# ShioMisaka/fce-yolo

Hardware: AMD Instinct MI355X
Metric: images/sec/GPU @ 640x640 bs=32, yolo11n-fce; fraction of fp16 MFMA roofline (higher is better)
Workload: dtype fp16; 1 GPU; yolo11n-fce detection inference (forward + decode + NMS) @ 640x640, 32 images/GPU; model=yolo11n-fce, global_batch=32, imgsz=640, parallelism=dp1, batches_in_flight=4, distinct_inputs=5, hw_queues=8, forward_launch=hipgraph

## Files before the change

### fce-yolo_amd/csrc/detect_cls.hip

```cpp
#include <algorithm>

#include "mfma_stage.h"

namespace fce {

static __device__ __attribute__((aligned(16))) _Float16 g_dc_zero[8];

constexpr int dc_max(int a, int b) { return a > b ? a : b; }

template <int C0, int C3, int NCLS, int TH, int TW, int NW>
struct DcG {
  static constexpr int NT = NW * 64;
  static constexpr int K0 = C0 / 8, K3 = C3 / 8;
  static constexpr int XW = TW + 4, XR = (TH + 4) * XW;
  static constexpr int RW = TW + 2, R1 = (TH + 2) * RW;
  static constexpr int NC = TH * TW;
  static constexpr int sX = K0, s1 = K0 | 1, s3 = K3 | 1;
  static constexpr int NF1 = (R1 + 15) / 16, NF2 = (NC + 15) / 16;
  static constexpr int MF1 = (NF1 + NW - 1) / NW, MF2 = (NF2 + NW - 1) / NW;
  static constexpr int CT3 = (C3 + 15) / 16, CTN = (NCLS + 15) / 16;
  static constexpr int NS1 = (K0 + 3) / 4, NS2 = (K3 + 3) / 4;
  static constexpr int W1 = CT3 * NS1 * 64, W2 = CT3 * NS2 * 64, W3 = CTN * NS2 * 64;
  static constexpr int OW2 = W1, OW3 = W1 + W2, OD = W1 + W2 + W3;
  static constexpr int ND = 9 * (C0 + C3);
  static constexpr int BD1 = 0, BP1 = C0, BD2 = BP1 + CT3 * 16, BP2 = BD2 + C3, BC = BP2 + CT3 * 16, NB = BC + CTN * 16;
  static constexpr int OB = OD + ND / 4;
  static constexpr int OP = OB + (NB + 3) / 4;
  static constexpr int PSZ = dc_max(R1 * s1, NC * s3);
  static constexpr int OQ = OP + PSZ;
  static constexpr int QX = XR * K0, QT = R1 * K3;
  static constexpr int QSZ = dc_max(dc_max(2 * QX, 2 * QT), NC * s3);
  static constexpr int TOTAL = OQ + QSZ;
  static constexpr size_t LDS = size_t(TOTAL) * 16;
  static constexpr int NXE = (XR * K0 + NT - 1) / NT;
  static constexpr int NPG3 = NT / K3;
  static constexpr int MINB = (LDS <= 80 * 1024 && NW == 4) ? 2 : 1;
  static_assert(C0 % 8 == 0 && C3 % 8 == 0 && NT % K0 == 0 && NPG3 > 0, "detect cls fused: channel alignment");
};

struct DclsArgs {
  const _Float16* x;
  int xcs;
  int H, W, tiles_x, tiles_y, ntiles;
  const float* dw[2];
  const h8* pw[3];
  int nalloc[3];
  const float* b[5];
  float* pred;
  unsigned long long* best;
  int A, a0;
  int diag;
};

__device__ __forceinline__ void dc_tile(const DclsArgs& a, int TH, int TW, int t, int& n, int& y0, int& x0) {
  const int tx = t % a.tiles_x;
  t /= a.tiles_x;
  const int ty = t % a.tiles_y;
  n = t / a.tiles_y;
  y0 = ty * TH;
  x0 = tx * TW;
}

typedef float f2 __attribute__((ext_vector_type(2)));
__device__ __forceinline__ h8 dc_dw(const f4* img, int plane, int p00, int rw, int k, int ch, int iy, int H,
                                    const float (&wk)[9][8], const float (&bz)[8]) {
  f2 acc[4];
#pragma unroll
  for (int j = 0; j < 4; ++j) acc[j] = f2{bz[2 * j], bz[2 * j + 1]};
#pragma unroll
  for (int ky = 0; ky < 3; ++ky) {
    const int yy = iy - 1 + ky;
    if (yy < 0 || yy >= H) continue;
#pragma unroll
    for (int kx = 0; kx < 3; ++kx) {
      const int u = (p00 + ky * rw + kx) * k + ch;
      const f4 lo = img[u], hi = img[plane + u];
      const float* w = wk[ky * 3 + kx];
      acc[0] = __builtin_elementwise_fma(f2{lo[0], lo[1]}, f2{w[0], w[1]}, acc[0]);
      acc[1] = __builtin_elementwise_fma(f2{lo[2], lo[3]}, f2{w[2], w[3]}, acc[1]);
      acc[2] = __builtin_elementwise_fma(f2{hi[0], hi[1]}, f2{w[4], w[5]}, acc[2]);
      acc[3] = __builtin_elementwise_fma(f2{hi[2], hi[3]}, f2{w[6], w[7]}, acc[3]);
    }
  }
  h8 o;
#pragma unroll
  for (int j = 0; j < 8; ++j) o[j] = (_Float16)fpin(silu(acc[j >> 1][j & 1]));
  return o;
}

__device__ __forceinline__ void dc_weights(const float* tab, int c, int ch, const float* bias, float (&wk)[9][8],
                                           float (&bz)[8]) {
#pragma unroll
  for (int t = 0; t < 9; ++t) {
    const f4 w0 = *reinterpret_cast<const f4*>(tab + t * c + ch * 8);
    const f4 w1 = *reinterpret_cast<const f4*>(tab + t * c + ch * 8 + 4);
#pragma unroll
    for (int j = 0; j < 4; ++j) {
      wk[t][j] = w0[j];
      wk[t][j + 4] = w1[j];
    }
  }
  const f4 b0 = *reinterpret_cast<const f4*>(bias + ch * 8);
  const f4 b1 = *reinterpret_cast<const f4*>(bias + ch * 8 + 4);
#pragma unroll
  for (int j = 0; j < 4; ++j) {
    bz[j] = b0[j];
    bz[j + 4] = b1[j];
  }
}

template <int C0, int C3, int NCLS, int TH, int TW, int NW>
__global__ __launch_bounds__(NW * 64, (DcG<C0, C3, NCLS, TH, TW, NW>::MINB)) void detect_cls_fused_kernel(DclsArgs a) {
  using G = DcG<C0, C3, NCLS, TH, TW, NW>;
  extern __shared__ __attribute__((aligned(16))) h8 sm[];
  const int tid = threadIdx.x, lane = tid & 63, wave = tid >> 6, col = lane & 15, grp = lane >> 4;
  const int NG = gridDim.x, bi = blockIdx.x;
  const int t_begin = int(int64_t(bi) * a.ntiles / NG), t_end = int(int64_t(bi + 1) * a.ntiles / NG);
  if (t_begin >= t_end) return;

  h8 xr[G::NXE];
  auto load_x = [&](int t) {
    int n, y0, x0;
    dc_tile(a, TH, TW, t, n, y0, x0);
#pragma unroll
    for (int k = 0; k < G::NXE; ++k) {
      const int e = tid + k * G::NT, pos = e / G::K0, ch = e - pos * G::K0;
      const int r = pos / G::XW, c = pos - r * G::XW;
      const int iy = y0 - 2 + r, ix = x0 - 2 + c;
      const bool in = pos < G::XR && iy >= 0 && iy < a.H && ix >= 0 && ix < a.W;
      const _Float16* src = in ? a.x + nhwc_off(n, iy, ix, a.H, a.W, a.xcs) + ch * 8 : g_dc_zero;
      xr[k] = *reinterpret_cast<const h8*>(src);
    }
  };
  load_x(t_begin);
  {
    stage_copy_frags(sm, a.pw[0], G::CT3, G::NS1, a.nalloc[0], G::NT);
    stage_copy_frags(sm + G::OW2, a.pw[1], G::CT3, G::NS2, a.nalloc[1], G::NT);
    stage_copy_frags(sm + G::OW3, a.pw[2], G::CTN, G::NS2, a.nalloc[2], G::NT);
    float* d = reinterpret_cast<float*>(sm + G::OD);
    for (int e = tid; e < 9 * C0; e += G::NT) d[e] = a.dw[0][e];
    for (int e = tid; e < 9 * C3; e += G::NT) d[9 * C0 + e] = a.dw[1][e];
    float* bs = reinterpret_cast<float*>(sm + G::OB);
    for (int e = tid; e < G::NB; e += G::NT) {
      float v;
      if (e < G::BP1) v = a.b[0][e];
      else if (e < G::BD2) v = e - G::BP1 < C3 ? a.b[1][e - G::BP1] : 0.f;
      else if (e < G::BP2) v = a.b[2][e - G::BD2];
      else if (e < G::BC) v = e - G::BP2 < C3 ? a.b[3][e - G::BP2] : 0.f;
      else v = e - G::BC < NCLS ? a.b[4][e - G::BC] : 0.f;
      bs[e] = v;
    }
  }
  __syncthreads();

  const float* dwt = reinterpret_cast<const float*>(sm + G::OD);
  const float* bias = reinterpret_cast<const float*>(sm + G::OB);
  h8* P = sm + G::OP;
  h8* Q = sm + G::OQ;
  _Float16* Qh = reinterpret_cast<_Float16*>(Q);
  f4* Qf = reinterpret_cast<f4*>(Q);
  const h8 zero8 = {0, 0, 0, 0, 0, 0, 0, 0};
  uint64_t clk[7] = {0, 0, 0, 0, 0, 0, 0}, tprev = a.diag ? __builtin_amdgcn_s_memtime() : 0;
  auto tick = [&](int k) {
    if (a.diag) {
      const uint64_t tn = __builtin_amdgcn_s_memtime();
      clk[k] += tn - tprev;
      tprev = tn;
    }
  };

  for (int t = t_begin; t < t_end; ++t) {
    int n, y0, x0;
    dc_tile(a, TH, TW, t, n, y0, x0);
#pragma unroll
    for (int k = 0; k < G::NXE; ++k) {
      const int e = tid + k * G::NT, pos = e / G::K0;
      if (pos < G::XR) {
        const h8 v = xr[k];
        Qf[e] = f4{(float)v[0], (float)v[1], (float)v[2], (float)v[3]};
        Qf[G::QX + e] = f4{(float)v[4], (float)v[5], (float)v[6], (float)v[7]};
      }
    }
    tick(0);
    if (t + 1 < t_end) load_x(t + 1);
    stage_barrier();
    tick(1);
    {
      const int ch = tid % G::K0;
      float wk[9][8], bz[8];
      dc_weights(dwt, C0, ch, bias + G::BD1, wk, bz);
      for (int pos = tid / G::K0; pos < G::R1; pos += G::NT / G::K0) {
        const int r = pos / G::RW, c = pos - r * G::RW;
        const int iy = y0 - 1 + r, ix = x0 - 1 + c;
        h8 o = zero8;
        if (iy >= 0 && iy < a.H && ix >= 0 && ix < a.W) o = dc_dw(Qf, G::QX, r * G::XW + c, G::XW, G::K0, ch, iy, a.H, wk, bz);
        P[pos * G::s1 + ch] = o;
      }
    }
    stage_barrier();
    tick(2);
    {
      int pq[G::MF1];
#pragma unroll
      for (int i = 0; i < G::MF1; ++i) pq[i] = min((wave + NW * i) * 16 + col, G::R1 - 1) * G::s1;
      auto bl = [&](int i, int st) -> h8 {
        const int cc = st * 4 + grp;
        return cc < G::K0 ? P[pq[i] + cc] : zero8;
      };
      auto epi = [&](int i, int ct, const f4& acc) {
        const int q = (wave + NW * i) * 16 + col, co0 = ct * 16 + grp * 4;
        if (q >= G::R1 || co0 >= C3) return;
        const int r = q / G::RW, c = q - r * G::RW;
        const int iy = y0 - 1 + r, ix = x0 - 1 + c;
        float v[4];
#pragma unroll
        for (int j = 0; j < 4; ++j) v[j] = silu(acc[j] + bias[G::BP1 + co0 + j]);
        const h4 o = h4_of(v);
        const bool in = iy >= 0 && iy < a.H && ix >= 0 && ix < a.W;
        Qf[(co0 & 4 ? G::QT : 0) + q * G::K3 + (co0 >> 3)] =
            in ? f4{(float)o[0], (float)o[1], (float)o[2], (float)o[3]} : f4{0.f, 0.f, 0.f, 0.f};
      };
      mfma_stage<G::MF1, G::CT3, G::NS1>(sm + lane, bl, epi);
    }
    stage_barrier();
    tick(3);
    if (tid < G::NPG3 * G::K3) {
      const int ch = tid % G::K3;
      float wk[9][8], bz[8];
      dc_weights(dwt + 9 * C0, C3, ch, bias + G::BD2, wk, bz);
      for (int pos = tid / G::K3; pos < G::NC; pos += G::NPG3) {
        const int r = pos / TW, c = pos - r * TW;
        const int iy = y0 + r, ix = x0 + c;
        h8 o = zero8;
        if (iy < a.H && ix < a.W) o = dc_dw(Qf, G::QT, r * G::RW + c, G::RW, G::K3, ch, iy, a.H, wk, bz);
        P[pos * G::s3 + ch] = o;
      }
    }
    stage_barrier();
    tick(4);
    {
      int pq[G::MF2];
#pragma unroll
      for (int i = 0; i < G::MF2; ++i) pq[i] = min((wave + NW * i) * 16 + col, G::NC - 1) * G::s3;
      auto bl = [&](int i, int st) -> h8 {
        const int cc = st * 4 + grp;
        return cc < G::K3 ? P[pq[i] + cc] : zero8;
      };
      auto epi = [&](int i, int ct, const f4& acc) {
        const int q = (wave + NW * i) * 16 + col, co0 = ct * 16 + grp * 4;
        if (q >= G::NC || co0 >= C3) return;
        float v[4];
#pragma unroll
        for (int j = 0; j < 4; ++j) v[j] = silu(acc[j] + bias[G::BP2 + co0 + j]);
        *reinterpret_cast<h4*>(Qh + (q * G::s3) * 8 + co0) = h4_of(v);
      };
      mfma_stage<G::MF2, G::CT3, G::NS2>(sm + G::OW2 + lane, bl, epi);
    }
    stage_barrier();
    tick(5);
    {
      int pq[G::MF2];
#pragma unroll
      for (int i = 0; i < G::MF2; ++i) pq[i] = min((wave + NW * i) * 16 + col, G::NC - 1) * G::s3;
      unsigned long long bk[G::MF2];
#pragma unroll
      for (int i = 0; i < G::MF2; ++i) bk[i] = 0ull;
      auto bl = [&](int i, int st) -> h8 {
        const int cc = st * 4 + grp;
        return cc < G::K3 ? Q[pq[i] + cc] : zero8;
      };
      auto epi = [&](int i, int ct, const f4& acc) {
        const int q = (wave + NW * i) * 16 + col, co0 = ct * 16 + grp * 4;
        if (q >= G::NC) return;
        const int r = q / TW, c = q - r * TW;
        const int iy = y0 + r, ix = x0 + c;
        if (iy >= a.H || ix >= a.W) return;
        float* o = a.pred + (int64_t(n) * (4 + NCLS) + 4 + co0) * a.A + a.a0 + iy * a.W + ix;
        const int nv = min(4, NCLS - co0);
#pragma unroll
        for (int j = 0; j < 4; ++j)
          if (j < nv) {
            const float sc = sigmoidf_(acc[j] + bias[G::BC + co0 + j]);
            o[int64_t(j) * a.A] = sc;
            const unsigned long long key =
                (uint64_t(__float_as_uint(sc)) << 32) | uint64_t(0xFFFFFFFFu - uint32_t(co0 + j));
            bk[i] = key > bk[i] ? key : bk[i];
          }
      };
      mfma_stage<G::MF2, G::CTN, G::NS2>(sm + G::OW3 + lane, bl, epi);
      if (a.best) {
#pragma unroll
        for (int i = 0; i < G::MF2; ++i) {
          unsigned long long k = bk[i];
          const unsigned long long k16 = __shfl_xor(k, 16);
          k = k16 > k ? k16 : k;
          const unsigned long long k32 = __shfl_xor(k, 32);
          k = k32 > k ? k32 : k;
          const int q = (wave + NW * i) * 16 + col;
          const int r = q / TW, c = q - r * TW;
          if (grp == 0 && q < G::NC && y0 + r < a.H && x0 + c < a.W && k)
            atomicMax(a.best + int64_t(n) * a.A + a.a0 + (y0 + r) * a.W + x0 + c, k);
        }
      }
    }
    stage_barrier();
    tick(6);
  }
  if (a.diag && blockIdx.x == 0 && threadIdx.x == 0) {
    const unsigned long long nt = (unsigned long long)(t_end - t_begin);
    printf("detect cls fused diag: %llu tiles, clocks per tile: x->lds %llu, x-issue+barrier %llu, dw1 %llu, pw1 %llu, "
           "dw2 %llu, pw2 %llu, cls %llu\n", nt, (unsigned long long)clk[0] / nt, (unsigned long long)clk[1] / nt,
           (unsigned long long)clk[2] / nt, (unsigned long long)clk[3] / nt, (unsigned long long)clk[4] / nt,
           (unsigned long long)clk[5] / nt, (unsigned long long)clk[6] / nt);
  }
}

struct DcInst {
  int c0, c3, nc;
};
static constexpr DcInst kDcInsts[] = {{64, 80, 80}, {128, 80, 80}};

template <int C0, int C3, int NCLS, int TH, int TW, int NW>
static int dc_launch(const DclsArgs& a0, int N, hipStream_t s) {
  using G = DcG<C0, C3, NCLS, TH, TW, NW>;
  static_assert(G::LDS <= 160 * 1024, "detect cls fused: LDS over 160 KiB");
  auto k = detect_cls_fused_kernel<C0, C3, NCLS, TH, TW, NW>;
  static const bool big = hipFuncSetAttribute(reinterpret_cast<const void*>(k),
                                              hipFuncAttributeMaxDynamicSharedMemorySize, 160 * 1024) == hipSuccess;
  if (!big && G::LDS > 64 * 1024) return fail(FCE_ERR_HIP, "detect cls fused: cannot opt in to >64 KiB LDS");
  DclsArgs a = a0;
  a.tiles_x = (a.W + TW - 1) / TW;
  a.tiles_y = (a.H + TH - 1) / TH;
  const int64_t tiles = int64_t(a.tiles_x) * a.tiles_y * N;
  if (tiles == 0) return FCE_OK;
  FCE_CHECK(tiles < (int64_t(1) << 30), "detect cls fused: grid too large");
  a.ntiles = int(tiles);
  static int cus = 0;
  if (!cus) {
    int dev = 0;
    if (hipGetDevice(&dev) != hipSuccess || hipDeviceGetAttribute(&cus, hipDeviceAttributeMultiprocessorCount, dev) != hipSuccess)
      cus = 256;
  }
  int occ = 0;
  if (hipOccupancyMaxActiveBlocksPerMultiprocessor(&occ, k, G::NT, G::LDS) != hipSuccess || occ < 1) occ = 1;
  const int grid = int(std::min<int64_t>(a.ntiles, int64_t(cus) * occ));
  FCE_LAUNCH(k, dim3(unsigned(grid)), dim3(G::NT), G::LDS, s, a);
  return launch_status("detect_cls_fused_kernel");
}

static bool dc_tile_env(const char* name, const char* v) {
  const char* e = getenv(name);
  return e && strcmp(e, v) == 0;
}

static int dc_dispatch(int inst, const DclsArgs& a, int N, hipStream_t s) {
  const char* name = inst == 0 ? "FCE_DCLS_TILE_64" : "FCE_DCLS_TILE_128";
  const char* env = getenv(name);
  const bool set = env && *env;
  if (inst == 0) {
    if (!set || dc_tile_env(name, "8,16,8")) return dc_launch<64, 80, 80, 8, 16, 8>(a, N, s);
    if (dc_tile_env(name, "8,16,4")) return dc_launch<64, 80, 80, 8, 16, 4>(a, N, s);
    if (dc_tile_env(name, "8,8,4")) return dc_launch<64, 80, 80, 8, 8, 4>(a, N, s);
  } else {
    if (!set || dc_tile_env(name, "8,8,8")) return dc_launch<128, 80, 80, 8, 8, 8>(a, N, s);
    if (dc_tile_env(name, "8,8,4")) return dc_launch<128, 80, 80, 8, 8, 4>(a, N, s);
  }
  return fail(FCE_ERR_INVALID, std::string(name) + ": not a tile of this instantiation");
}

static int dc_inst(const fce_dcls_desc& d) {
  for (int i = 0; i < int(sizeof(kDcInsts) / sizeof(kDcInsts[0])); ++i)
    if (kDcInsts[i].c0 == d.c0 && kDcInsts[i].c3 == d.c3 && kDcInsts[i].nc == d.nc) return i;
  return -1;
}

bool detect_cls_fused_ok(const fce_dcls_desc& d) { return dc_inst(d) >= 0; }

int detect_cls_fused(const fce_dcls_desc& d, const fce_tensor& x, const fce_detect_epi& e, hipStream_t s) {
  const int inst = dc_inst(d);
  FCE_CHECK(inst >= 0, "detect cls fused: unsupported channel configuration");
  FCE_CHECK(x.layout == FCE_NHWC && x.dtype == FCE_F16 && x.c == d.c0, "detect cls fused: NHWC f16 view of c0 channels");
  FCE_CHECK(x.cstride % 8 == 0 && x.coff % 8 == 0, "detect cls fused: aligned channel slice");
  FCE_CHECK(e.pred && e.part == 1 && e.nc == d.nc && e.anchor_offset >= 0 &&
                int64_t(e.anchor_offset) + int64_t(x.h) * x.w <= e.anchors,
            "detect cls fused: the cls epilogue of this level (part 1, nc, anchors)");
  for (int i = 0; i < 5; ++i) FCE_CHECK(d.w[i] && d.b[i], "detect cls fused: null weights");
  DclsArgs a{};
  a.x = static_cast<const _Float16*>(x.data) + x.coff;
  a.xcs = x.cstride;
  a.H = x.h;
  a.W = x.w;
  a.dw[0] = static_cast<const float*>(d.w[0]);
  a.dw[1] = static_cast<const float*>(d.w[2]);
  a.pw[0] = static_cast<const h8*>(d.w[1]);
  a.pw[1] = static_cast<const h8*>(d.w[3]);
  a.pw[2] = static_cast<const h8*>(d.w[4]);
  a.nalloc[0] = stage_nalloc(d.c0, 1);
  a.nalloc[1] = stage_nalloc(d.c3, 1);
  a.nalloc[2] = stage_nalloc(d.c3, 1);
  for (int i = 0; i < 5; ++i) a.b[i] = d.b[i];
  a.pred = e.pred;
  a.best = e.best;
  a.A = e.anchors;
  a.a0 = e.anchor_offset;
  {
    const char* de = getenv("FCE_DCLS_DIAG");
    a.diag = de && atoi(de) != 0;
  }
  return dc_dispatch(inst, a, x.n, s);
}

}
```

### fce-yolo_amd/csrc/fused.hip

```cpp
#include <algorithm>

#include "mfma_stage.h"

namespace fce {

static __device__ __attribute__((aligned(16))) _Float16 g_c3_zero[8];

template <int CIN, int C, int CM, int COUT, int TH, int TW, int NW>
struct C3G {
  static constexpr int R2W = TW + 4, R2 = (TH + 4) * R2W;
  static constexpr int R1W = TW + 2, R1 = (TH + 2) * R1W;
  static constexpr int NC = TH * TW;
  static constexpr int NF1 = (R2 + 15) / 16, NF2 = (R1 + 15) / 16, NF4 = (NC + 15) / 16;
  static constexpr int MF1 = (NF1 + NW - 1) / NW, MF2 = (NF2 + NW - 1) / NW, MF4 = (NF4 + NW - 1) / NW;
  static constexpr int CT1 = 2 * C / 16, CT2 = (CM + 15) / 16, CT3 = (C + 15) / 16, CT4 = (COUT + 15) / 16;
  static constexpr bool F2 = C % 32 == 0, F3 = CM % 32 == 0;
  static constexpr int NS1 = CIN / 32, NS2 = (9 * (C / 8) + 3) / 4, NS3 = (9 * (CM / 8) + 3) / 4,
                       NS4 = (3 * C / 8 + 3) / 4;
  static constexpr int sT = (2 * C / 8) | 1, sH = (CM / 8) | 1, sM = (C / 8) | 1;
  static constexpr int W1 = CT1 * NS1 * 64, W2 = CT2 * NS2 * 64, W3 = CT3 * NS3 * 64, W4 = CT4 * NS4 * 64;
  static constexpr int OW2 = W1, OW3 = W1 + W2, OW4 = W1 + W2 + W3, OB = W1 + W2 + W3 + W4;
  static constexpr int B2 = CT1 * 16, B3 = B2 + CT2 * 16, B4 = B3 + CT3 * 16, NB = B4 + CT4 * 16;
  static constexpr int OT = OB + NB / 4, OH = OT + R2 * sT, OM = OH + R1 * sH, TOTAL = OM + NC * sM;
  static constexpr size_t LDS = size_t(TOTAL) * 16;
  static_assert(CIN % 32 == 0 && C % 8 == 0 && CM % 8 == 0 && COUT % 8 == 0, "c3k2 fused: channel alignment");
};

struct C3k2Args {
  const _Float16* x;
  int xcs;
  _Float16* y;
  int ycs;
  int H, W, tiles_x, tiles_y, ntiles;
  const h8* w[4];
  int nalloc[4];
  const float* b[4];
  int diag;
};

__device__ __forceinline__ void c3_act(const float* bias, int ct, int grp, const f4& acc, float (&v)[4]) {
  const int co0 = ct * 16 + grp * 4;
#pragma unroll
  for (int j = 0; j < 4; ++j) v[j] = silu(acc[j] + bias[co0 + j]);
}

template <bool FAST, int CPT>
__device__ __forceinline__ void c3_kstep(int st, int grp, int& tap, int& cc, bool& ok) {
  if (FAST) {
    tap = st % 9;
    cc = (st / 9) * 4 + grp;
    ok = true;
  } else {
    const int k = st * 4 + grp;
    tap = k / CPT;
    cc = k - tap * CPT;
    ok = tap < 9;
  }
}

__device__ __forceinline__ void c3_tile(const C3k2Args& a, int TH, int TW, int t, int& n, int& y0, int& x0) {
  const int tx = t % a.tiles_x;
  t /= a.tiles_x;
  const int ty = t % a.tiles_y;
  n = t / a.tiles_y;
  y0 = ty * TH;
  x0 = tx * TW;
}

template <int CIN, int C, int CM, int COUT, int TH, int TW, int NW, bool YB>
__global__ __launch_bounds__(NW * 64, 2) void c3k2_fused_kernel(C3k2Args a) {
  using G = C3G<CIN, C, CM, COUT, TH, TW, NW>;
  extern __shared__ __attribute__((aligned(16))) h8 sm[];
  const int lane = threadIdx.x & 63, wave = threadIdx.x >> 6, col = lane & 15, grp = lane >> 4;
  const int NG = gridDim.x, bi = blockIdx.x;
  const int t_begin = int(int64_t(bi) * a.ntiles / NG), t_end = int(int64_t(bi + 1) * a.ntiles / NG);
  if (t_begin >= t_end) return;

  h8 xb[G::MF1][G::NS1];
  auto load_x = [&](int t) {
    int n, y0, x0;
    c3_tile(a, TH, TW, t, n, y0, x0);
    const _Float16* zl = g_c3_zero;
#pragma unroll
    for (int i = 0; i < G::MF1; ++i) {
      const int q = (wave + NW * i) * 16 + col;
      const int r = q / G::R2W, cq = q - r * G::R2W;
      const int iy = y0 - 2 + r, ix = x0 - 2 + cq;
      const bool in = q < G::R2 && iy >= 0 && iy < a.H && ix >= 0 && ix < a.W;
      const _Float16* src = a.x + (in ? nhwc_off(n, iy, ix, a.H, a.W, a.xcs) + grp * 8 : 0);
#pragma unroll
      for (int s = 0; s < G::NS1; ++s) xb[i][s] = *reinterpret_cast<const h8*>(in ? src + s * 32 : zl);
    }
  };
  load_x(t_begin);
  {
    const int wofs[4] = {0, G::OW2, G::OW3, G::OW4}, cts[4] = {G::CT1, G::CT2, G::CT3, G::CT4};
    const int nss[4] = {G::NS1, G::NS2, G::NS3, G::NS4}, couts[4] = {2 * C, CM, C, COUT};
    const int bofs[4] = {0, G::B2, G::B3, G::B4};
    float* bias = reinterpret_cast<float*>(sm + G::OB);
#pragma unroll
    for (int s = 0; s < 4; ++s) {
      stage_copy_frags(sm + wofs[s], a.w[s], cts[s], nss[s], a.nalloc[s], NW * 64);
      for (int e = int(threadIdx.x); e < cts[s] * 16; e += NW * 64) bias[bofs[s] + e] = e < couts[s] ? a.b[s][e] : 0.f;
    }
  }
  __syncthreads();

  const float* bias = reinterpret_cast<const float*>(sm + G::OB);
  _Float16* T = reinterpret_cast<_Float16*>(sm + G::OT);
  _Float16* Hh = reinterpret_cast<_Float16*>(sm + G::OH);
  _Float16* Mm = reinterpret_cast<_Float16*>(sm + G::OM);
  const h8* Tin = sm + G::OT;
  const h8* Hin = sm + G::OH;
  const h8* Min = sm + G::OM;
  uint64_t clk[6] = {0, 0, 0, 0, 0, 0}, tprev = a.diag ? __builtin_amdgcn_s_memtime() : 0;
  auto tick = [&](int k) {
    if (a.diag) {
      const uint64_t tn = __builtin_amdgcn_s_memtime();
      clk[k] += tn - tprev;
      tprev = tn;
    }
  };

  for (int t = t_begin; t < t_end; ++t) {
    int n, y0, x0;
    c3_tile(a, TH, TW, t, n, y0, x0);
    {
      auto bl = [&](int i, int st) -> h8 { return xb[i][st]; };
      auto epi = [&](int i, int ct, const f4& acc) {
        const int q = (wave + NW * i) * 16 + col;
        if (q >= G::R2) return;
        const int r = q / G::R2W, cq = q - r * G::R2W;
        const int iy = y0 - 2 + r, ix = x0 - 2 + cq;
        float v[4];
        c3_act(bias, ct, grp, acc, v);
        h4 o = h4_of(v);
        if (!(iy >= 0 && iy < a.H && ix >= 0 && ix < a.W)) o = h4{0, 0, 0, 0};
        *reinterpret_cast<h4*>(T + (q * G::sT) * 8 + ct * 16 + grp * 4) = o;
      };
      mfma_stage<G::MF1, G::CT1, G::NS1>(sm + lane, bl, epi);
    }
    tick(0);
    if (t + 1 < t_end) load_x(t + 1);
    tick(1);
    stage_barrier();
    {
      int pb[G::MF2];
#pragma unroll
      for (int i = 0; i < G::MF2; ++i) {
        const int q = min((wave + NW * i) * 16 + col, G::R1 - 1);
        const int r = q / G::R1W, cq = q - r * G::R1W;
        pb[i] = r * G::R2W + cq;
      }
      auto bl = [&](int i, int st) -> h8 {
        int tap, cc;
        bool ok;
        c3_kstep<G::F2, C / 8>(st, grp, tap, cc, ok);
        const int ky = tap / 3, kx = tap - ky * 3;
        return ok ? Tin[(pb[i] + ky * G::R2W + kx) * G::sT + C / 8 + cc] : h8{0, 0, 0, 0, 0, 0, 0, 0};
      };
      auto epi = [&](int i, int ct, const f4& acc) {
        const int q = (wave + NW * i) * 16 + col;
        if (q >= G::R1 || ct * 16 + grp * 4 >= CM) return;
        const int r = q / G::R1W, cq = q - r * G::R1W;
        const int iy = y0 - 1 + r, ix = x0 - 1 + cq;
        float v[4];
        c3_act(bias + G::B2, ct, grp, acc, v);
        h4 o = h4_of(v);
        if (!(iy >= 0 && iy < a.H && ix >= 0 && ix < a.W)) o = h4{0, 0, 0, 0};
        *reinterpret_cast<h4*>(Hh + (q * G::sH) * 8 + ct * 16 + grp * 4) = o;
      };
      mfma_stage<G::MF2, G::CT2, G::NS2>(sm + G::OW2 + lane, bl, epi);
    }
    tick(2);
    stage_barrier();
    {
      int pb[G::MF4];
#pragma unroll
      for (int i = 0; i < G::MF4; ++i) {
        const int q = min((wave + NW * i) * 16 + col, G::NC - 1);
        const int r = q / TW, cq = q - r * TW;
        pb[i] = r * G::R1W + cq;
      }
      auto bl = [&](int i, int st) -> h8 {
        int tap, cc;
        bool ok;
        c3_kstep<G::F3, CM / 8>(st, grp, tap, cc, ok);
        const int ky = tap / 3, kx = tap - ky * 3;
        return ok ? Hin[(pb[i] + ky * G::R1W + kx) * G::sH + cc] : h8{0, 0, 0, 0, 0, 0, 0, 0};
      };
      auto epi = [&](int i, int ct, const f4& acc) {
        const int q = (wave + NW * i) * 16 + col;
        const int co0 = ct * 16 + grp * 4;
        if (q >= G::NC || co0 >= C) return;
        const int r = q / TW, cq = q - r * TW;
        float v[4];
        c3_act(bias + G::B3, ct, grp, acc, v);
        const h4 rv = *reinterpret_cast<const h4*>(T + (((r + 2) * G::R2W + cq + 2) * G::sT) * 8 + C + co0);
#pragma unroll
        for (int j = 0; j < 4; ++j) v[j] = fpin(v[j] + (float)rv[j]);
        *reinterpret_cast<h4*>(Mm + (q * G::sM) * 8 + co0) = h4_of(v);
      };
      mfma_stage<G::MF4, G::CT3, G::NS3>(sm + G::OW3 + lane, bl, epi);
    }
    tick(3);
    stage_barrier();
    {
      int pt[G::MF4], pm[G::MF4];
#pragma unroll
      for (int i = 0; i < G::MF4; ++i) {
        const int q = min((wave + NW * i) * 16 + col, G::NC - 1);
        const int r = q / TW, cq = q - r * TW;
        pt[i] = ((r + 2) * G::R2W + cq + 2) * G::sT;
        pm[i] = q * G::sM - 2 * C / 8;
      }
      auto bl = [&](int i, int st) -> h8 {
        const int cc = st * 4 + grp;
        if (cc >= 3 * C / 8) return h8{0, 0, 0, 0, 0, 0, 0, 0};
        return cc < 2 * C / 8 ? Tin[pt[i] + cc] : Min[pm[i] + cc];
      };
      const uint32_t img = uint32_t(a.H) * uint32_t(a.W) * uint32_t(a.ycs);
      const __amdgpu_buffer_rsrc_t yr = out_rsrc(a.y + int64_t(n) * img, img * 2u);
      auto epi = [&](int i, int ct, const f4& acc) {
        const int q = (wave + NW * i) * 16 + col;
        const int r = q / TW, cq = q - r * TW;
        const int iy = y0 + r, ix = x0 + cq;
        const bool ok = q < G::NC && ct * 16 + grp * 4 < COUT && iy < a.H && ix < a.W;
        if (!YB && !ok) return;
        float v[4];
        c3_act(bias + G::B4, ct, grp, acc, v);
        const int off = (iy * a.W + ix) * a.ycs + ct * 16 + grp * 4;
        if constexpr (YB) store_h4_or_drop(yr, ok, uint32_t(off) * 2u, h4_of(v));
        else *reinterpret_cast<h4*>(a.y + int64_t(n) * img + off) = h4_of(v);
      };
      mfma_stage<G::MF4, G::CT4, G::NS4>(sm + G::OW4 + lane, bl, epi);
    }
    tick(4);
    stage_barrier();
    tick(5);
  }
  if (a.diag && blockIdx.x == 0 && threadIdx.x == 0) {
    const unsigned long long nt = (unsigned long long)(t_end - t_begin);
    printf("c3k2 fused diag: %llu tiles, clocks per tile: stage1 %llu, x-issue %llu, stage2 %llu, stage3 %llu, "
           "stage4 %llu, last barrier %llu\n", nt, (unsigned long long)clk[0] / nt, (unsigned long long)clk[1] / nt,
           (unsigned long long)clk[2] / nt, (unsigned long long)clk[3] / nt, (unsigned long long)clk[4] / nt,
           (unsigned long long)clk[5] / nt);
  }
}

struct C3Inst {
  int cin, c, cm, cout;
};
static constexpr C3Inst kC3Insts[] = {{32, 16, 8, 64}, {64, 32, 16, 128}, {32, 32, 16, 64}};

template <int CIN, int C, int CM, int COUT, int TH, int TW, int NW, bool YB>
static int c3_launch(const C3k2Args& a0, int H, int W, int N, hipStream_t s) {
  using G = C3G<CIN, C, CM, COUT, TH, TW, NW>;
  static_assert(G::LDS <= 160 * 1024, "c3k2 fused: LDS over 160 KiB");
  auto k = c3k2_fused_kernel<CIN, C, CM, COUT, TH, TW, NW, YB>;
  static const bool big = hipFuncSetAttribute(reinterpret_cast<const void*>(k),
                                              hipFuncAttributeMaxDynamicSharedMemorySize, 160 * 1024) == hipSuccess;
  if (!big && G::LDS > 64 * 1024) return fail(FCE_ERR_HIP, "c3k2 fused: cannot opt in to >64 KiB LDS");
  C3k2Args a = a0;
  a.tiles_x = (W + TW - 1) / TW;
  a.tiles_y = (H + TH - 1) / TH;
  const int64_t tiles = int64_t(a.tiles_x) * a.tiles_y * N;
  if (tiles == 0) return FCE_OK;
  FCE_CHECK(tiles < (int64_t(1) << 30), "c3k2 fused: grid too large");
  a.ntiles = int(tiles);
  static int cus = 0;
  if (!cus) {
    int dev = 0;
    if (hipGetDevice(&dev) != hipSuccess || hipDeviceGetAttribute(&cus, hipDeviceAttributeMultiprocessorCount, dev) != hipSuccess)
      cus = 256;
  }
  int occ = 0;
  if (hipOccupancyMaxActiveBlocksPerMultiprocessor(&occ, k, NW * 64, G::LDS) != hipSuccess || occ < 1) occ = 1;
  {
    static const int cap = [] {
      const char* e = getenv("FCE_C3K2_OCC");
      return e ? atoi(e) : 0;
    }();
    if (cap > 0) occ = std::min(occ, cap);
  }
  const int grid = int(std::min<int64_t>(a.ntiles, int64_t(cus) * occ));
  FCE_LAUNCH(k, dim3(unsigned(grid)), dim3(NW * 64), G::LDS, s, a);
  return launch_status("c3k2_fused_kernel");
}

template <int CIN, int C, int CM, int COUT>
static int c3_launch_cfg(const C3k2Args& a, int H, int W, int N, hipStream_t s) {
  const char* env = getenv("FCE_C3K2_TILE");
  bool wide = W >= 128;
  if (env && *env) {
    if (strcmp(env, "8,16,4") == 0) wide = true;
    else if (strcmp(env, "4,40,8") == 0) wide = false;
    else return fail(FCE_ERR_INVALID, "FCE_C3K2_TILE: only \"8,16,4\" or \"4,40,8\"");
  }
  const char* yst = getenv("FCE_C3K2_YSTORE");
  bool yb = COUT <= 64;
  if (yst && *yst) {
    if (strcmp(yst, "buf") == 0) yb = true;
    else if (strcmp(yst, "global") == 0) yb = false;
    else return fail(FCE_ERR_INVALID, "FCE_C3K2_YSTORE: only \"buf\" or \"global\"");
  }
  if (wide) return yb ? c3_launch<CIN, C, CM, COUT, 8, 16, 4, true>(a, H, W, N, s) : c3_launch<CIN, C, CM, COUT, 8, 16, 4, false>(a, H, W, N, s);
  return yb ? c3_launch<CIN, C, CM, COUT, 4, 40, 8, true>(a, H, W, N, s) : c3_launch<CIN, C, CM, COUT, 4, 40, 8, false>(a, H, W, N, s);
}

static int c3_inst(const fce_c3k2_desc& d) {
  for (int i = 0; i < int(sizeof(kC3Insts) / sizeof(kC3Insts[0])); ++i)
    if (kC3Insts[i].cin == d.cin && kC3Insts[i].c == d.c && kC3Insts[i].cm == d.c_mid && kC3Insts[i].cout == d.cout)
      return i;
  return -1;
}

bool c3k2_fused_ok(const fce_c3k2_desc& d) { return c3_inst(d) >= 0; }

int c3k2_fused(const fce_c3k2_desc& d, const fce_tensor& x, const fce_tensor& y, hipStream_t s) {
  const int inst = c3_inst(d);
  FCE_CHECK(inst >= 0, "c3k2 fused: unsupported channel configuration");
  FCE_CHECK(x.layout == FCE_NHWC && y.layout == FCE_NHWC && x.dtype == FCE_F16 && y.dtype == FCE_F16,
            "c3k2 fused: NHWC f16 views");
  FCE_CHECK(x.c == d.cin && y.c == d.cout && x.n == y.n && x.h == y.h && x.w == y.w, "c3k2 fused: shape mismatch");
  FCE_CHECK(x.cstride % 8 == 0 && x.coff % 8 == 0 && y.cstride % 4 == 0 && y.coff % 4 == 0,
            "c3k2 fused: aligned channel slices");
  for (int i = 0; i < 4; ++i) FCE_CHECK(d.w[i] && d.b[i], "c3k2 fused: null weights");
  C3k2Args a{};
  a.x = static_cast<const _Float16*>(x.data) + x.coff;
  a.xcs = x.cstride;
  a.y = static_cast<_Float16*>(y.data) + y.coff;
  a.ycs = y.cstride;
  a.H = x.h;
  a.W = x.w;
  const int cins[4] = {d.cin, d.c, d.c_mid, 3 * d.c}, ks[4] = {1, 3, 3, 1};
  for (int i = 0; i < 4; ++i) {
    a.w[i] = static_cast<const h8*>(d.w[i]);
    a.b[i] = d.b[i];
    a.nalloc[i] = stage_nalloc(cins[i], ks[i]);
  }
  {
    const char* de = getenv("FCE_C3K2_DIAG");
    a.diag = de && atoi(de) != 0;
  }
  switch (inst) {
    case 0: return c3_launch_cfg<32, 16, 8, 64>(a, x.h, x.w, x.n, s);
    case 1: return c3_launch_cfg<64, 32, 16, 128>(a, x.h, x.w, x.n, s);
    default: return c3_launch_cfg<32, 32, 16, 64>(a, x.h, x.w, x.n, s);
  }
}

}
```

### fce-yolo_amd/csrc/mfma_stage.h

```cpp
#pragma once
#include "common.h"

namespace fce {

__device__ __forceinline__ void stage_barrier() {
  asm volatile("s_waitcnt lgkmcnt(0)" ::: "memory");
  __builtin_amdgcn_s_barrier();
  asm volatile("" ::: "memory");
}

__device__ __forceinline__ h4 h4_of(const float (&v)[4]) {
  return h4{(_Float16)fpin(v[0]), (_Float16)fpin(v[1]), (_Float16)fpin(v[2]), (_Float16)fpin(v[3])};
}

template <int MF, int CT, int NS, typename BL, typename EPI>
__device__ __forceinline__ void mfma_stage(const h8* wl, BL bl, EPI epi) {
  f4 acc[MF][CT];
#pragma unroll
  for (int i = 0; i < MF; ++i)
#pragma unroll
    for (int ct = 0; ct < CT; ++ct) acc[i][ct] = f4{0.f, 0.f, 0.f, 0.f};
  h8 av[2][CT], bv[2][MF];
  auto load = [&](int st, h8 (&a)[CT], h8 (&b)[MF]) {
#pragma unroll
    for (int ct = 0; ct < CT; ++ct) a[ct] = wl[(ct * NS + st) * 64];
#pragma unroll
    for (int i = 0; i < MF; ++i) b[i] = bl(i, st);
  };
  load(0, av[0], bv[0]);
#pragma unroll
  for (int st = 0; st < NS; ++st) {
    if (st + 1 < NS) load(st + 1, av[(st + 1) & 1], bv[(st + 1) & 1]);
    __builtin_amdgcn_sched_barrier(0);
#pragma unroll
    for (int i = 0; i < MF; ++i)
#pragma unroll
      for (int ct = 0; ct < CT; ++ct)
        acc[i][ct] = __builtin_amdgcn_mfma_f32_16x16x32_f16(av[st & 1][ct], bv[st & 1][i], acc[i][ct], 0, 0, 0);
    __builtin_amdgcn_sched_barrier(0);
  }
#pragma unroll
  for (int i = 0; i < MF; ++i)
#pragma unroll
    for (int ct = 0; ct < CT; ++ct) epi(i, ct, acc[i][ct]);
}

__device__ __forceinline__ void stage_copy_frags(h8* dst, const h8* src, int ct_n, int ns, int nalloc, int nt) {
  const int nfr = ct_n * ns * 64;
  for (int e0 = int(threadIdx.x); e0 < nfr; e0 += 4 * nt) {
    h8 v[4];
#pragma unroll
    for (int u = 0; u < 4; ++u) {
      const int e = e0 + u * nt;
      const int k = e >> 6, ct = k / ns, stp = k - ct * ns;
      if (e < nfr) v[u] = src[(size_t(ct) * nalloc + stp) * 64 + (e & 63)];
    }
#pragma unroll
    for (int u = 0; u < 4; ++u) {
      const int e = e0 + u * nt;
      if (e < nfr) dst[e] = v[u];
    }
  }
}

inline int stage_nalloc(int cin, int k) {
  const int nsteps = (k * k * (cin / 8) + 3) / 4;
  return ((nsteps + 7) & ~7) + 8;
}

}
```

Baseline: 39570 images/sec.

## Carry halo rows between vertically adjacent tiles in fused C3k2 kernel

Measured after the change: 39370 images/sec. No clear change (-0.5%).

```diff
diff --git a/fce-yolo_amd/csrc/detect_cls.hip b/fce-yolo_amd/csrc/detect_cls.hip
--- a/fce-yolo_amd/csrc/detect_cls.hip
+++ b/fce-yolo_amd/csrc/detect_cls.hip
@@ -343,7 +343,10 @@
   }
   int occ = 0;
   if (hipOccupancyMaxActiveBlocksPerMultiprocessor(&occ, k, G::NT, G::LDS) != hipSuccess || occ < 1) occ = 1;
-  const int grid = int(std::min<int64_t>(a.ntiles, int64_t(cus) * occ));
+  int grid = int(std::min<int64_t>(a.ntiles, int64_t(cus) * occ));
+  const int cap = fused_grid_cap();
+  if (cap < 0) return fail(FCE_ERR_INVALID, "FCE_FUSED_GRID: a positive block count");
+  if (cap > 0) grid = std::min(grid, cap);
   FCE_LAUNCH(k, dim3(unsigned(grid)), dim3(G::NT), G::LDS, s, a);
   return launch_status("detect_cls_fused_kernel");
 }
diff --git a/fce-yolo_amd/csrc/fused.hip b/fce-yolo_amd/csrc/fused.hip
--- a/fce-yolo_amd/csrc/fused.hip
+++ b/fce-yolo_amd/csrc/fused.hip
@@ -23,6 +23,12 @@
   static constexpr int B2 = CT1 * 16, B3 = B2 + CT2 * 16, B4 = B3 + CT3 * 16, NB = B4 + CT4 * 16;
   static constexpr int OT = OB + NB / 4, OH = OT + R2 * sT, OM = OH + R1 * sH, TOTAL = OM + NC * sM;
   static constexpr size_t LDS = size_t(TOTAL) * 16;
+  static constexpr int Q1C = 4 * R2W, Q2C = 2 * R1W;
+  static constexpr int NF1C = (R2 - Q1C + 15) / 16, NF2C = (R1 - Q2C + 15) / 16;
+  static constexpr int MF1C = (NF1C + NW - 1) / NW, MF2C = (NF2C + NW - 1) / NW;
+  static constexpr int KT = Q1C * sT, KH = Q2C * sH;
+  static constexpr int NKT = (KT + NW * 64 - 1) / (NW * 64), NKH = (KH + NW * 64 - 1) / (NW * 64);
+  static_assert(TH >= 4, "c3k2 fused: the kept rows and their new home must not overlap");
   static_assert(CIN % 32 == 0 && C % 8 == 0 && CM % 8 == 0 && COUT % 8 == 0, "c3k2 fused: channel alignment");
 };
 
@@ -58,16 +64,25 @@
   }
 }
 
+template <bool COLS>
 __device__ __forceinline__ void c3_tile(const C3k2Args& a, int TH, int TW, int t, int& n, int& y0, int& x0) {
-  const int tx = t % a.tiles_x;
-  t /= a.tiles_x;
-  const int ty = t % a.tiles_y;
-  n = t / a.tiles_y;
+  int tx, ty;
+  if (COLS) {
+    ty = t % a.tiles_y;
+    t /= a.tiles_y;
+    tx = t % a.tiles_x;
+    n = t / a.tiles_x;
+  } else {
+    tx = t % a.tiles_x;
+    t /= a.tiles_x;
+    ty = t % a.tiles_y;
+    n = t / a.tiles_y;
+  }
   y0 = ty * TH;
   x0 = tx * TW;
 }
 
-template <int CIN, int C, int CM, int COUT, int TH, int TW, int NW, bool YB>
+template <int CIN, int C, int CM, int COUT, int TH, int TW, int NW, bool YB, bool CARRY>
 __global__ __launch_bounds__(NW * 64, 2) void c3k2_fused_kernel(C3k2Args a) {
   using G = C3G<CIN, C, CM, COUT, TH, TW, NW>;
   extern __shared__ __attribute__((aligned(16))) h8 sm[];
@@ -77,13 +92,15 @@
   if (t_begin >= t_end) return;
 
   h8 xb[G::MF1][G::NS1];
-  auto load_x = [&](int t) {
+  auto load_x = [&](int t, bool carried) {
     int n, y0, x0;
-    c3_tile(a, TH, TW, t, n, y0, x0);
+    c3_tile<CARRY>(a, TH, TW, t, n, y0, x0);
     const _Float16* zl = g_c3_zero;
+    const int q0 = CARRY && carried ? G::Q1C : 0;
 #pragma unroll
     for (int i = 0; i < G::MF1; ++i) {
-      const int q = (wave + NW * i) * 16 + col;
+      if (CARRY && i >= G::MF1C && carried) continue;
+      const int q = q0 + (wave + NW * i) * 16 + col;
       const int r = q / G::R2W, cq = q - r * G::R2W;
       const int iy = y0 - 2 + r, ix = x0 - 2 + cq;
       const bool in = q < G::R2 && iy >= 0 && iy < a.H && ix >= 0 && ix < a.W;
@@ -92,7 +109,8 @@
       for (int s = 0; s < G::NS1; ++s) xb[i][s] = *reinterpret_cast<const h8*>(in ? src + s * 32 : zl);
     }
   };
-  load_x(t_begin);
+  auto is_carried = [&](int t) { return CARRY && t > t_begin && t % a.tiles_y != 0; };
+  load_x(t_begin, false);
   {
     const int wofs[4] = {0, G::OW2, G::OW3, G::OW4}, cts[4] = {G::CT1, G::CT2, G::CT3, G::CT4};
     const int nss[4] = {G::NS1, G::NS2, G::NS3, G::NS4}, couts[4] = {2 * C, CM, C, COUT};
@@ -122,13 +140,20 @@
     }
   };
 
+  h8 kt[G::NKT];
+#pragma unroll
+  for (int k = 0; k < G::NKT; ++k) kt[k] = h8{0, 0, 0, 0, 0, 0, 0, 0};
   for (int t = t_begin; t < t_end; ++t) {
     int n, y0, x0;
-    c3_tile(a, TH, TW, t, n, y0, x0);
-    {
+    c3_tile<CARRY>(a, TH, TW, t, n, y0, x0);
+    const bool carried = is_carried(t), carry_next = t + 1 < t_end && is_carried(t + 1);
+    int q1 = CARRY && carried ? G::Q1C : 0, q2 = CARRY && carried ? G::Q2C : 0;
+    if (CARRY) asm volatile("" : "+s"(q1), "+s"(q2));
+    auto stage1 = [&](auto mf, int q0) __attribute__((always_inline)) {
+      constexpr int MF = decltype(mf)::value;
       auto bl = [&](int i, int st) -> h8 { return xb[i][st]; };
       auto epi = [&](int i, int ct, const f4& acc) {
-        const int q = (wave + NW * i) * 16 + col;
+        const int q = q0 + (wave + NW * i) * 16 + col;
         if (q >= G::R2) return;
         const int r = q / G::R2W, cq = q - r * G::R2W;
         const int iy = y0 - 2 + r, ix = x0 - 2 + cq;
@@ -138,17 +163,28 @@
         if (!(iy >= 0 && iy < a.H && ix >= 0 && ix < a.W)) o = h4{0, 0, 0, 0};
         *reinterpret_cast<h4*>(T + (q * G::sT) * 8 + ct * 16 + grp * 4) = o;
       };
-      mfma_stage<G::MF1, G::CT1, G::NS1>(sm + lane, bl, epi);
+      mfma_stage<MF, G::CT1, G::NS1>(sm + lane, bl, epi);
+    };
+    if (CARRY && carried) {
+#pragma unroll
+      for (int k = 0; k < G::NKT; ++k) {
+        const int u = int(threadIdx.x) + k * NW * 64;
+        if (u < G::KT) sm[G::OT + u] = kt[k];
+      }
+      stage1(std::integral_constant<int, G::MF1C>{}, q1);
+    } else {
+      stage1(std::integral_constant<int, G::MF1>{}, q1);
     }
     tick(0);
-    if (t + 1 < t_end) load_x(t + 1);
+    if (t + 1 < t_end) load_x(t + 1, carry_next);
     tick(1);
     stage_barrier();
-    {
-      int pb[G::MF2];
-#pragma unroll
-      for (int i = 0; i < G::MF2; ++i) {
-        const int q = min((wave + NW * i) * 16 + col, G::R1 - 1);
+    auto stage2 = [&](auto mf, int q0) __attribute__((always_inline)) {
+      constexpr int MF = decltype(mf)::value;
+      int pb[MF];
+#pragma unroll
+      for (int i = 0; i < MF; ++i) {
+        const int q = min(q0 + (wave + NW * i) * 16 + col, G::R1 - 1);
         const int r = q / G::R1W, cq = q - r * G::R1W;
         pb[i] = r * G::R2W + cq;
       }
@@ -160,7 +196,7 @@
         return ok ? Tin[(pb[i] + ky * G::R2W + kx) * G::sT + C / 8 + cc] : h8{0, 0, 0, 0, 0, 0, 0, 0};
       };
       auto epi = [&](int i, int ct, const f4& acc) {
-        const int q = (wave + NW * i) * 16 + col;
+        const int q = q0 + (wave + NW * i) * 16 + col;
         if (q >= G::R1 || ct * 16 + grp * 4 >= CM) return;
         const int r = q / G::R1W, cq = q - r * G::R1W;
         const int iy = y0 - 1 + r, ix = x0 - 1 + cq;
@@ -170,8 +206,10 @@
         if (!(iy >= 0 && iy < a.H && ix >= 0 && ix < a.W)) o = h4{0, 0, 0, 0};
         *reinterpret_cast<h4*>(Hh + (q * G::sH) * 8 + ct * 16 + grp * 4) = o;
       };
-      mfma_stage<G::MF2, G::CT2, G::NS2>(sm + G::OW2 + lane, bl, epi);
-    }
+      mfma_stage<MF, G::CT2, G::NS2>(sm + G::OW2 + lane, bl, epi);
+    };
+    if (CARRY && carried) stage2(std::integral_constant<int, G::MF2C>{}, q2);
+    else stage2(std::integral_constant<int, G::MF2>{}, q2);
     tick(2);
     stage_barrier();
     {
@@ -205,6 +243,13 @@
     }
     tick(3);
     stage_barrier();
+    if (CARRY && carry_next) {
+#pragma unroll
+      for (int k = 0; k < G::NKH; ++k) {
+        const int u = int(threadIdx.x) + k * NW * 64;
+        if (u < G::KH) sm[G::OH + u] = Hin[TH * G::R1W * G::sH + u];
+      }
+    }
     {
       int pt[G::MF4], pm[G::MF4];
 #pragma unroll
@@ -235,6 +280,13 @@
       };
       mfma_stage<G::MF4, G::CT4, G::NS4>(sm + G::OW4 + lane, bl, epi);
     }
+    if (CARRY && carry_next) {
+#pragma unroll
+      for (int k = 0; k < G::NKT; ++k) {
+        const int u = int(threadIdx.x) + k * NW * 64;
+        if (u < G::KT) kt[k] = Tin[TH * G::R2W * G::sT + u];
+      }
+    }
     tick(4);
     stage_barrier();
     tick(5);
@@ -253,11 +305,11 @@
 };
 static constexpr C3Inst kC3Insts[] = {{32, 16, 8, 64}, {64, 32, 16, 128}, {32, 32, 16, 64}};
 
-template <int CIN, int C, int CM, int COUT, int TH, int TW, int NW, bool YB>
+template <int CIN, int C, int CM, int COUT, int TH, int TW, int NW, bool YB, bool CARRY>
 static int c3_launch(const C3k2Args& a0, int H, int W, int N, hipStream_t s) {
   using G = C3G<CIN, C, CM, COUT, TH, TW, NW>;
   static_assert(G::LDS <= 160 * 1024, "c3k2 fused: LDS over 160 KiB");
-  auto k = c3k2_fused_kernel<CIN, C, CM, COUT, TH, TW, NW, YB>;
+  auto k = c3k2_fused_kernel<CIN, C, CM, COUT, TH, TW, NW, YB, CARRY>;
   static const bool big = hipFuncSetAttribute(reinterpret_cast<const void*>(k),
                                               hipFuncAttributeMaxDynamicSharedMemorySize, 160 * 1024) == hipSuccess;
   if (!big && G::LDS > 64 * 1024) return fail(FCE_ERR_HIP, "c3k2 fused: cannot opt in to >64 KiB LDS");
@@ -283,10 +335,23 @@
     }();
     if (cap > 0) occ = std::min(occ, cap);
   }
-  const int grid = int(std::min<int64_t>(a.ntiles, int64_t(cus) * occ));
+  int grid = int(std::min<int64_t>(a.ntiles, int64_t(cus) * occ));
+  const int cap = fused_grid_cap();
+  if (cap < 0) return fail(FCE_ERR_INVALID, "FCE_FUSED_GRID: a positive block count");
+  if (cap > 0) grid = std::min(grid, cap);
   FCE_LAUNCH(k, dim3(unsigned(grid)), dim3(NW * 64), G::LDS, s, a);
   return launch_status("c3k2_fused_kernel");
 }
+
+template <int CIN, int C, int CM, int COUT, int TH, int TW, int NW>
+static int c3_launch_yc(bool yb, bool carry, const C3k2Args& a, int H, int W, int N, hipStream_t s) {
+  if (yb) return carry ? c3_launch<CIN, C, CM, COUT, TH, TW, NW, true, true>(a, H, W, N, s)
+                       : c3_launch<CIN, C, CM, COUT, TH, TW, NW, true, false>(a, H, W, N, s);
+  return carry ? c3_launch<CIN, C, CM, COUT, TH, TW, NW, false, true>(a, H, W, N, s)
+               : c3_launch<CIN, C, CM, COUT, TH, TW, NW, false, false>(a, H, W, N, s);
+}
+
+static bool c3_carry_default(int c, bool wide) { return !wide && c == 32; }
 
 template <int CIN, int C, int CM, int COUT>
 static int c3_launch_cfg(const C3k2Args& a, int H, int W, int N, hipStream_t s) {
@@ -304,8 +369,11 @@
     else if (strcmp(yst, "global") == 0) yb = false;
     else return fail(FCE_ERR_INVALID, "FCE_C3K2_YSTORE: only \"buf\" or \"global\"");
   }
-  if (wide) return yb ? c3_launch<CIN, C, CM, COUT, 8, 16, 4, true>(a, H, W, N, s) : c3_launch<CIN, C, CM, COUT, 8, 16, 4, false>(a, H, W, N, s);
-  return yb ? c3_launch<CIN, C, CM, COUT, 4, 40, 8, true>(a, H, W, N, s) : c3_launch<CIN, C, CM, COUT, 4, 40, 8, false>(a, H, W, N, s);
+  const int cs = fused_switch("FCE_C3K2_CARRY");
+  if (cs == -2) return fail(FCE_ERR_INVALID, "FCE_C3K2_CARRY: only \"0\" or \"1\"");
+  const bool carry = cs < 0 ? c3_carry_default(C, wide) : cs == 1;
+  if (wide) return c3_launch_yc<CIN, C, CM, COUT, 8, 16, 4>(yb, carry, a, H, W, N, s);
+  return c3_launch_yc<CIN, C, CM, COUT, 4, 40, 8>(yb, carry, a, H, W, N, s);
 }
 
 static int c3_inst(const fce_c3k2_desc& d) {
diff --git a/fce-yolo_amd/csrc/mfma_stage.h b/fce-yolo_amd/csrc/mfma_stage.h
--- a/fce-yolo_amd/csrc/mfma_stage.h
+++ b/fce-yolo_amd/csrc/mfma_stage.h
@@ -63,6 +63,22 @@
   }
 }
 
+inline int fused_grid_cap() {
+  const char* e = getenv("FCE_FUSED_GRID");
+  if (!e || !*e) return 0;
+  char* end = nullptr;
+  const long v = strtol(e, &end, 10);
+  return (*end || v < 1 || v > (1L << 30)) ? -1 : int(v);
+}
+
+inline int fused_switch(const char* name) {
+  const char* e = getenv(name);
+  if (!e || !*e) return -1;
+  if (strcmp(e, "0") == 0) return 0;
+  if (strcmp(e, "1") == 0) return 1;
+  return -2;
+}
+
 inline int stage_nalloc(int cin, int k) {
   const int nsteps = (k * k * (cin / 8) + 3) / 4;
   return ((nsteps + 7) & ~7) + 8;
```
